# SobeyMIL/MVOC

Hardware: AMD Instinct MI355X
Metric: UNet3D denoising steps/sec, 16x512^2 frames, inversion+compose (higher is better)
Workload: dtype f16

## Files before the change

### mvoc_amd/csrc/attention.hip

```cpp
#include <stdlib.h>

#include "common.h"

namespace {

typedef __fp16 fp16x4_t __attribute__((__vector_size__(4 * sizeof(__fp16))));
template <int D> struct FlashPitch { static constexpr int K = 2 * D + 16, V = D == 64 ? 192 : 320; };

struct AttnArgs {
  const half_t *q, *k, *v;
  half_t* out;
  long q_bs, q_ts, k_bs, k_ts, v_bs, v_ts, o_bs, o_ts;
  int nbatch, heads, tq, tk, kv_bdiv, causal;
  float scale_log2;
  long v2_off, o2_off;
  int qblocks;
};

__device__ __forceinline__ int vt_slot_group(int key) {
  return ((((key >> 5) * 2 + ((key >> 4) & 1)) * 2) + ((key >> 2) & 1));
}
__device__ __forceinline__ int vt_slot_elem(int key) { return ((key >> 3) & 1) * 4 + (key & 3); }

constexpr float FLASH_THR = 8.0f;

typedef float f32x2 __attribute__((ext_vector_type(2)));
__device__ __forceinline__ float flash_xhalf_max(float x) {
  const unsigned u = __builtin_bit_cast(unsigned, x);
  const auto sw = __builtin_amdgcn_permlane32_swap(u, u, false, false);
  return fmaxf(__builtin_bit_cast(float, (unsigned)sw[0]), __builtin_bit_cast(float, (unsigned)sw[1]));
}

template <int D, int NV>
#ifndef FLASH_MINW
#define FLASH_MINW 4
#endif
__global__ __launch_bounds__(256, (D == 64 && NV == 1) ? FLASH_MINW : 1) void flash_kernel(const AttnArgs p) {
  constexpr int KPITCH = FlashPitch<D>::K, VPITCH = FlashPitch<D>::V;
  constexpr int ND = D / 16, NT = D / 32, CPK = D / 8, NCH = 64 * CPK / 256;
  __shared__ __attribute__((aligned(16))) char smem[64 * KPITCH + NV * 64 * VPITCH];
  char* Ks = smem;
  char* Vs = smem + 64 * KPITCH;
  const int tid = threadIdx.x, lane = tid & 63;
  const int wave = __builtin_amdgcn_readfirstlane(tid >> 6);
  const int r = lane & 31, h = lane >> 5;
  const unsigned logical = xcd_remap(blockIdx.x, gridDim.x);
  const unsigned qb_ = logical % (unsigned)p.qblocks, hb_ = logical / (unsigned)p.qblocks;
  const int head = (int)(hb_ % (unsigned)p.heads), b = (int)(hb_ / (unsigned)p.heads);
  const int q0 = (int)qb_ * 128 + wave * 32;

  const half_t* qp = p.q + (long)b * p.q_bs + head * D;
  const int qrow = min(q0 + r, p.tq - 1);
  half8_t qf[ND];
#pragma unroll
  for (int s = 0; s < ND; ++s) qf[s] = *reinterpret_cast<const half8_t*>(qp + (long)qrow * p.q_ts + 16 * s + 8 * h);

  const char* kb = reinterpret_cast<const char*>(p.k + (long)(b / p.kv_bdiv) * p.k_bs + head * D);
  const char* vb = reinterpret_cast<const char*>(p.v + (long)(b / p.kv_bdiv) * p.v_bs + head * D);
  const unsigned k_rb = (unsigned)p.k_ts * 2u, v_rb = (unsigned)p.v_ts * 2u;
  unsigned koff[NCH], voff[NCH];
#pragma unroll
  for (int i = 0; i < NCH; ++i) {
    const int c = tid + i * 256;
    koff[i] = (unsigned)(c / CPK) * k_rb + (unsigned)(c % CPK) * 16u;
    voff[i] = (unsigned)(c / CPK) * v_rb + (unsigned)(c % CPK) * 16u;
  }

  f32x16 ot[NV][NT];
#pragma unroll
  for (int v = 0; v < NV; ++v)
#pragma unroll
    for (int dt = 0; dt < NT; ++dt)
#pragma unroll
      for (int e = 0; e < 16; ++e) ot[v][dt][e] = 0.f;
  float mrun = -INFINITY, lrun = 0.f;

  const int ntiles = (p.tk + 63) / 64;
  half8_t kreg[NCH], vreg[NV][NCH];
  auto gload = [&](int kt) {
    const char* kt_ = kb + (size_t)kt * 64u * k_rb;
    const char* vt_ = vb + (size_t)kt * 64u * v_rb;
    const bool ragged = __builtin_amdgcn_readfirstlane(kt * 64 + 64 > p.tk);
#pragma unroll
    for (int i = 0; i < NCH; ++i) {
      unsigned ko = koff[i], vo = voff[i];
      if (ragged) {
        const int c = tid + i * 256;
        const unsigned row = (unsigned)min(c / CPK, p.tk - 1 - kt * 64);
        ko = row * k_rb + (unsigned)(c % CPK) * 16u;
        vo = row * v_rb + (unsigned)(c % CPK) * 16u;
      }
      kreg[i] = *reinterpret_cast<const half8_t*>(kt_ + ko);
#pragma unroll
      for (int v = 0; v < NV; ++v) vreg[v][i] = *reinterpret_cast<const half8_t*>(vt_ + (size_t)v * (size_t)p.v2_off * 2u + vo);
    }
  };
  gload(0);
  for (int kt = 0; kt < ntiles; ++kt) {
    __syncthreads();
#pragma unroll
    for (int i = 0; i < NCH; ++i) {
      const int c = tid + i * 256;
      const int key = c / CPK, dc = c % CPK;
      *reinterpret_cast<half8_t*>(Ks + key * KPITCH + dc * 16) = kreg[i];
#pragma unroll
      for (int v = 0; v < NV; ++v)
        *reinterpret_cast<half8_t*>(Vs + v * 64 * VPITCH + key * VPITCH + dc * 16) = vreg[v][i];
    }
    __syncthreads();
    if (kt + 1 < ntiles) gload(kt + 1);

    f32x16 st[2];
#pragma unroll
    for (int t = 0; t < 2; ++t) {
#pragma unroll
      for (int e = 0; e < 16; ++e) st[t][e] = 0.f;
#pragma unroll
      for (int s = 0; s < ND; ++s) {
        const half8_t kf = *reinterpret_cast<const half8_t*>(Ks + (32 * t + r) * KPITCH + (16 * s + 8 * h) * 2);
        st[t] = __builtin_amdgcn_mfma_f32_32x32x16_f16(kf, qf[s], st[t], 0, 0, 0);
      }
    }
    if (__builtin_amdgcn_readfirstlane((kt == ntiles - 1) && (p.tk & 63))) {
#pragma unroll
      for (int t = 0; t < 2; ++t)
#pragma unroll
        for (int e = 0; e < 16; ++e)
          if (kt * 64 + 32 * t + 8 * (e >> 2) + 4 * h + (e & 3) >= p.tk) st[t][e] = -INFINITY;
    }
    if (p.causal) {
#pragma unroll
      for (int t = 0; t < 2; ++t)
#pragma unroll
        for (int e = 0; e < 16; ++e)
          if (kt * 64 + 32 * t + 8 * (e >> 2) + 4 * h + (e & 3) > q0 + r) st[t][e] = -INFINITY;
    }
    float mx = st[0][0];
#pragma unroll
    for (int t = 0; t < 2; ++t)
#pragma unroll
      for (int e = 0; e < 16; ++e) mx = fmaxf(mx, st[t][e]);
    mx = flash_xhalf_max(mx);
    if (__any((mx - mrun) * p.scale_log2 > FLASH_THR)) {
      const float mnew = fmaxf(mrun, mx);
      const float alpha = __builtin_amdgcn_exp2f((mrun - mnew) * p.scale_log2);
      mrun = mnew;
      lrun *= alpha;
#pragma unroll
      for (int v = 0; v < NV; ++v)
#pragma unroll
        for (int dt = 0; dt < NT; ++dt)
#pragma unroll
          for (int e = 0; e < 16; ++e) ot[v][dt][e] *= alpha;
    }
    const f32x2 sc2 = {p.scale_log2, p.scale_log2}, mc2 = {-mrun * p.scale_log2, -mrun * p.scale_log2};
#pragma unroll
    for (int t = 0; t < 2; ++t)
#pragma unroll
      for (int e = 0; e < 16; e += 2) {
        const f32x2 a = __builtin_elementwise_fma(f32x2{st[t][e], st[t][e + 1]}, sc2, mc2);
        st[t][e] = __builtin_amdgcn_exp2f(a[0]);
        st[t][e + 1] = __builtin_amdgcn_exp2f(a[1]);
      }

#pragma unroll
    for (int t = 0; t < 2; ++t)
#pragma unroll
      for (int s = 0; s < 2; ++s) {
        half8_t pf;
#pragma unroll
        for (int j = 0; j < 8; ++j) pf[j] = (half_t)st[t][8 * s + j];
#pragma unroll
        for (int j = 0; j < 4; ++j) lrun = __builtin_amdgcn_fdot2(half2_t{pf[2 * j], pf[2 * j + 1]}, half2_t{(half_t)1.f, (half_t)1.f}, lrun, false);
        const int krow = 32 * t + 16 * s + 4 * h + ((lane & 15) >> 2);
#pragma unroll
        for (int v = 0; v < NV; ++v)
#pragma unroll
          for (int dt = 0; dt < NT; ++dt) {
            const char* va = Vs + v * 64 * VPITCH + krow * VPITCH + (32 * dt + 16 * ((lane >> 4) & 1) + 4 * (lane & 3)) * 2;
            const fp16x4_t lo = __builtin_amdgcn_ds_read_tr16_b64_v4f16((__attribute__((address_space(3))) fp16x4_t*)va);
            const fp16x4_t hi = __builtin_amdgcn_ds_read_tr16_b64_v4f16((__attribute__((address_space(3))) fp16x4_t*)(va + 8 * VPITCH));
            half8_t vf;
#pragma unroll
            for (int e = 0; e < 4; ++e) {
              vf[e] = (half_t)lo[e];
              vf[4 + e] = (half_t)hi[e];
            }
            ot[v][dt] = __builtin_amdgcn_mfma_f32_32x32x16_f16(vf, pf, ot[v][dt], 0, 0, 0);
          }
      }
  }
  const float ltot = lrun + __shfl_xor(lrun, 32);
  const float inv = 1.0f / ltot;
  int lane_e = tid;
  asm volatile("" : "+v"(lane_e));
  const int r_e = lane_e & 31, h_e = (lane_e >> 5) & 1;
  if (q0 + r_e < p.tq) {
#pragma unroll
    for (int v = 0; v < NV; ++v) {
      half_t* op = p.out + v * p.o2_off + (long)b * p.o_bs + (long)(q0 + r_e) * p.o_ts + head * D;
#pragma unroll
      for (int dt = 0; dt < NT; ++dt)
#pragma unroll
        for (int q = 0; q < 4; ++q) {
          half4_t o;
#pragma unroll
          for (int e = 0; e < 4; ++e) o[e] = (half_t)(ot[v][dt][q * 4 + e] * inv);
          *reinterpret_cast<half4_t*>(op + 32 * dt + 8 * q + 4 * h_e) = o;
        }
    }
  }
}

#define F3_BAR()                         \
  do {                                   \
    __builtin_amdgcn_sched_barrier(0);   \
    __builtin_amdgcn_s_barrier();        \
    __builtin_amdgcn_sched_barrier(0);   \
  } while (0)
#define F3_FENCE() __builtin_amdgcn_sched_barrier(0)
#define F3_GRP(V, T)                                   \
  do {                                                 \
    __builtin_amdgcn_sched_group_barrier(0x008, 1, 0); \
    __builtin_amdgcn_sched_group_barrier(0x002, V, 0); \
    __builtin_amdgcn_sched_group_barrier(0x400, T, 0); \
  } while (0)
#define F3_RD(R) __builtin_amdgcn_sched_group_barrier(0x100, R, 0)
#ifdef MVOC_F3_STAMPS
__device__ unsigned long long f3_dbg[8];
#define F3_STAMP(i)                                                                      \
  do {                                                                                   \
    unsigned long long t_;                                                               \
    asm volatile("s_memtime %0\n\ts_waitcnt lgkmcnt(0)" : "=s"(t_)::"memory");          \
    if (blockIdx.x == 0 && tid == 0) { f3_acc[i] += t_ - f3_last; }                      \
    f3_last = t_;                                                                        \
  } while (0)
#else
#define F3_STAMP(i)
#endif
typedef unsigned u32x4 __attribute__((ext_vector_type(4)));
__device__ __forceinline__ void f3_dma(const u32x4 rsrc, unsigned voff, unsigned lds) {
  unsigned keep;
  asm volatile("s_mov_b32 %0, m0\n\ts_mov_b32 m0, %2\n\ts_nop 0\n\tbuffer_load_dwordx4 %1, %3, 0 offen lds\n\ts_mov_b32 m0, %0"
               : "=&s"(keep) : "v"(voff), "s"(lds), "s"(rsrc) : "memory");
}
__device__ __forceinline__ u32x4 f3_rsrc(const void* base, unsigned bytes) {
  const unsigned long long a = (unsigned long long)base;
  u32x4 r;
  r[0] = __builtin_amdgcn_readfirstlane((unsigned)a);
  r[1] = __builtin_amdgcn_readfirstlane((unsigned)(a >> 32));
  r[2] = __builtin_amdgcn_readfirstlane(bytes);
  r[3] = 0x00020000u;
  return r;
}
template <int N>
__device__ __forceinline__ void f3_wait_vm() {
  asm volatile("s_waitcnt vmcnt(%0)" ::"n"(N) : "memory");
}
#ifndef F3_W1
#define F3_W1 3
#endif
template <int NV>
__global__ __launch_bounds__(256, NV == 1 ? F3_W1 : 2) void flash3_kernel(const AttnArgs p) {
  constexpr int D = 64, NS = (NV == 1 && F3_W1 == 2) ? 4 : 3, TILE = 8192 * (1 + NV), PCS = 2 + 2 * NV;
  __shared__ __attribute__((aligned(1024))) char smem[NS * TILE];
#ifdef MVOC_F3_STAMPS
  unsigned long long f3_acc[6] = {0, 0, 0, 0, 0, 0}, f3_last = 0, f3_t0, f3_r0;
#endif
  const int tid = threadIdx.x, lane = tid & 63;
  const int wave = __builtin_amdgcn_readfirstlane(tid >> 6);
  const int r = lane & 31, h = lane >> 5;
#ifdef MVOC_F3_STAMPS
  asm volatile("s_memtime %0\n\ts_memrealtime %1\n\ts_waitcnt lgkmcnt(0)" : "=s"(f3_t0), "=s"(f3_r0)::"memory");
  f3_last = f3_t0;
#endif
  const unsigned logical = xcd_remap(blockIdx.x, gridDim.x);
  const unsigned qb_ = logical % (unsigned)p.qblocks, hb_ = logical / (unsigned)p.qblocks;
  const int head = (int)(hb_ % (unsigned)p.heads), b = (int)(hb_ / (unsigned)p.heads);
  const int q0 = (int)qb_ * 128 + wave * 32;
  const int nt = (p.tk + 63) >> 6;

  const unsigned k_rb = (unsigned)p.k_ts * 2u, v_rb = (unsigned)p.v_ts * 2u;
  const half_t* kb = p.k + (long)(b / p.kv_bdiv) * p.k_bs + head * D;
  const half_t* vb = p.v + (long)(b / p.kv_bdiv) * p.v_bs + head * D;
  const u32x4 rs_k = f3_rsrc(kb, (unsigned)(p.tk - 1) * k_rb + 128u);
  const u32x4 rs_v0 = f3_rsrc(vb, (unsigned)(p.tk - 1) * v_rb + 128u);
  const u32x4 rs_v1 = f3_rsrc(vb + p.v2_off, (unsigned)(p.tk - 1) * v_rb + 128u);
  unsigned ksrc[2], vsrc[2];
#pragma unroll
  for (int j = 0; j < 2; ++j) {
    const int key_l = 16 * wave + 8 * j + (lane >> 3), pc = lane & 7;
    ksrc[j] = (unsigned)key_l * k_rb + (unsigned)((pc ^ ((key_l >> 1) & 7)) * 16);
    vsrc[j] = (unsigned)key_l * v_rb + (unsigned)((pc ^ (((key_l >> 1) & 1) << 2)) * 16);
  }
  const unsigned ktile = 64u * k_rb, vtile = 64u * v_rb;
  const unsigned lds0 = (unsigned)(size_t)(__attribute__((address_space(3))) char*)smem;
  auto issue = [&](int tile, int so) {
    const unsigned base = lds0 + (unsigned)so + (unsigned)wave * 2048u;
#pragma unroll
    for (int j = 0; j < 2; ++j) f3_dma(rs_k, ksrc[j] + (unsigned)tile * ktile, base + j * 1024);
#pragma unroll
    for (int v = 0; v < NV; ++v)
#pragma unroll
      for (int j = 0; j < 2; ++j) f3_dma(v ? rs_v1 : rs_v0, vsrc[j] + (unsigned)tile * vtile, base + 8192 * (1 + v) + j * 1024);
  };
  const half_t* qp = p.q + (long)b * p.q_bs + head * D;
  const int qrow = min(q0 + r, p.tq - 1);
  half8_t qf[4];
#pragma unroll
  for (int s = 0; s < 4; ++s) qf[s] = *reinterpret_cast<const half8_t*>(qp + (long)qrow * p.q_ts + 16 * s + 8 * h);
  asm volatile("s_nop 4" ::: "memory");
  F3_FENCE();
#pragma unroll
  for (int t = 0; t < NS - 1; ++t) issue(t, t * TILE);
  F3_FENCE();

  f32x16 ot[NV][2];
#pragma unroll
  for (int v = 0; v < NV; ++v)
#pragma unroll
    for (int dt = 0; dt < 2; ++dt)
#pragma unroll
      for (int e = 0; e < 16; ++e) ot[v][dt][e] = 0.f;
  float mrun = -INFINITY, lrun = 0.f;
  f32x16 sa[2], sb[2];
  f32x16 zero16;
#pragma unroll
  for (int e = 0; e < 16; ++e) zero16[e] = 0.f;

  int kfo[4];
#pragma unroll
  for (int s = 0; s < 4; ++s) kfo[s] = r * 128 + (((2 * s + h) ^ ((r >> 1) & 7)) * 16);
  const int vq = (lane & 15) >> 2;
  int vfo[2];
#pragma unroll
  for (int dt = 0; dt < 2; ++dt) vfo[dt] = 8192 + (4 * h + vq) * 128 + (((32 * ((lane >> 4) & 1) + 8 * (lane & 3))) | ((dt ^ ((vq >> 1) & 1)) << 6));

  f3_wait_vm<(NS - 2) * PCS>();
  F3_BAR();
#pragma unroll
  for (int t = 0; t < 2; ++t) {
    sa[t] = zero16;
#pragma unroll
    for (int s = 0; s < 4; ++s) {
      const half8_t kf = *reinterpret_cast<const half8_t*>(smem + kfo[s] + 4096 * t);
      sa[t] = __builtin_amdgcn_mfma_f32_32x32x16_f16(kf, qf[s], sa[t], 0, 0, 0);
    }
  }
  int o_v = 0, o_k = TILE, o_w = (NS - 1) * TILE;

  auto body = [&](f32x16(&cur)[2], f32x16(&nxt)[2], const int t) {
    F3_STAMP(4);
    f3_wait_vm<(NS - 3) * PCS>();
    F3_BAR();
    F3_STAMP(0);
    issue(t + NS - 1, o_w);
    F3_FENCE();
    F3_STAMP(1);
    const char* Kn = smem + o_k;
    const char* Vc = smem + o_v;
    if (__builtin_amdgcn_readfirstlane((t == nt - 1) && (p.tk & 63))) {
#pragma unroll
      for (int tt = 0; tt < 2; ++tt)
#pragma unroll
        for (int e = 0; e < 16; ++e)
          if (t * 64 + 32 * tt + 8 * (e >> 2) + 4 * h + (e & 3) >= p.tk) cur[tt][e] = -INFINITY;
    }
    F3_FENCE();
    half8_t kf[2][4];
#pragma unroll
    for (int s = 0; s < 2; ++s)
#pragma unroll
      for (int tt = 0; tt < 2; ++tt) kf[tt][s] = *reinterpret_cast<const half8_t*>(Kn + kfo[s] + 4096 * tt);
    half8_t pf[2];
    half8_t vf[3][NV][2];
    auto vread = [&](const int f) {
#pragma unroll
      for (int v = 0; v < NV; ++v)
#pragma unroll
        for (int dt = 0; dt < 2; ++dt) {
          const char* va = Vc + 8192 * v + vfo[dt] + (32 * (f >> 1) + 16 * (f & 1)) * 128;
          const fp16x4_t lo = __builtin_amdgcn_ds_read_tr16_b64_v4f16((__attribute__((address_space(3))) fp16x4_t*)va);
          const fp16x4_t hi = __builtin_amdgcn_ds_read_tr16_b64_v4f16((__attribute__((address_space(3))) fp16x4_t*)(va + 8 * 128));
#pragma unroll
          for (int e = 0; e < 4; ++e) {
            vf[f % 3][v][dt][e] = (half_t)lo[e];
            vf[f % 3][v][dt][4 + e] = (half_t)hi[e];
          }
        }
    };
    vread(0);
    F3_FENCE();
    auto smma = [&](const int i) {
      const int tt = i & 1, s_ = i >> 1;
      nxt[tt] = __builtin_amdgcn_mfma_f32_32x32x16_f16(kf[tt][s_], qf[s_], s_ == 0 ? zero16 : nxt[tt], 0, 0, 0);
    };
    auto pvmma = [&](const int f, const int dt) {
#pragma unroll
      for (int v = 0; v < NV; ++v) ot[v][dt] = __builtin_amdgcn_mfma_f32_32x32x16_f16(vf[f % 3][v][dt], pf[f & 1], ot[v][dt], 0, 0, 0);
    };
    float mx = fmaxf(cur[0][0], cur[0][1]);
#pragma unroll
    for (int tt = 0; tt < 2; ++tt)
#pragma unroll
      for (int e = tt ? 0 : 2; e < 16; e += 2) mx = __builtin_fmaxf(__builtin_fmaxf(mx, cur[tt][e]), cur[tt][e + 1]);
    smma(0); smma(1); smma(2);
    if constexpr (NV == 2) smma(3);
    mx = flash_xhalf_max(mx);
    if constexpr (NV == 1) { F3_GRP(6, 0); F3_GRP(6, 0); F3_GRP(6, 0); }
    else { F3_GRP(4, 0); F3_GRP(5, 0); F3_GRP(4, 0); F3_GRP(5, 0); }
    F3_STAMP(2);
    if (__any((mx - mrun) * p.scale_log2 > FLASH_THR)) {
      const float mnew = fmaxf(mrun, mx);
      const float alpha = __builtin_amdgcn_exp2f((mrun - mnew) * p.scale_log2);
      mrun = mnew;
      lrun *= alpha;
#pragma unroll
      for (int v = 0; v < NV; ++v)
#pragma unroll
        for (int dt = 0; dt < 2; ++dt)
#pragma unroll
          for (int e = 0; e < 16; ++e) ot[v][dt][e] *= alpha;
    }
    F3_FENCE();
    const f32x2 sc2 = {p.scale_log2, p.scale_log2}, mc2 = {-mrun * p.scale_log2, -mrun * p.scale_log2};
#pragma unroll
    for (int s = 2; s < 4; ++s)
#pragma unroll
      for (int tt = 0; tt < 2; ++tt) kf[tt][s] = *reinterpret_cast<const half8_t*>(Kn + kfo[s] + 4096 * tt);
#pragma unroll
    for (int f = 0; f < 4; ++f) {
      const int tt = f >> 1, s_ = f & 1;
      if (f < 3) vread(f + 1);
      half8_t& pn = pf[f & 1];
      float x[8];
#pragma unroll
      for (int j = 0; j < 8; j += 2) {
        const f32x2 a = __builtin_elementwise_fma(f32x2{cur[tt][8 * s_ + j], cur[tt][8 * s_ + j + 1]}, sc2, mc2);
        x[j] = __builtin_amdgcn_exp2f(a[0]);
        x[j + 1] = __builtin_amdgcn_exp2f(a[1]);
      }
#pragma unroll
      for (int j = 0; j < 8; ++j) pn[j] = (half_t)x[j];
#pragma unroll
      for (int j = 0; j < 4; ++j) lrun = __builtin_amdgcn_fdot2(half2_t{pn[2 * j], pn[2 * j + 1]}, half2_t{(half_t)1.f, (half_t)1.f}, lrun, false);
      if (f == 0) {
        smma(NV == 1 ? 3 : 4); smma(NV == 1 ? 4 : 5);
        if constexpr (NV == 2) { smma(6); smma(7); } else smma(5);
      } else {
        pvmma(f - 1, 0); pvmma(f - 1, 1);
        if constexpr (NV == 1) { if (f < 3) smma(5 + f); }
      }
    }
    pvmma(3, 0);
    pvmma(3, 1);
    if constexpr (NV == 1) {
      F3_RD(8); F3_GRP(5, 3); F3_GRP(5, 2); F3_GRP(5, 3);
      F3_RD(4); F3_GRP(5, 2); F3_GRP(5, 3); F3_GRP(5, 2);
      F3_RD(4); F3_GRP(5, 3); F3_GRP(5, 2); F3_GRP(5, 3);
      F3_GRP(5, 2); F3_GRP(5, 3); F3_GRP(5, 2); F3_GRP(5, 2);
    } else {
      F3_RD(12); F3_GRP(3, 2); F3_GRP(3, 2); F3_GRP(3, 2); F3_GRP(3, 2);
      F3_RD(8); F3_GRP(3, 2); F3_GRP(3, 2); F3_GRP(3, 2); F3_GRP(3, 2);
      F3_RD(8); F3_GRP(3, 2); F3_GRP(3, 2); F3_GRP(3, 2); F3_GRP(3, 2);
      F3_GRP(3, 2); F3_GRP(3, 2); F3_GRP(3, 2); F3_GRP(3, 2);
      F3_GRP(3, 0); F3_GRP(3, 0); F3_GRP(3, 0); F3_GRP(3, 0);
    }
    F3_FENCE();
    F3_STAMP(3);
    const int o_ = o_v; o_v = o_k;
    o_k = o_k + TILE == NS * TILE ? 0 : o_k + TILE;
    o_w = o_;
  };
#pragma unroll 1
  for (int t = 0;; t += 2) {
    body(sa, sb, t);
    if (t + 1 >= nt) break;
    body(sb, sa, t + 1);
    if (t + 2 >= nt) break;
  }
  f3_wait_vm<0>();
#ifdef MVOC_F3_STAMPS
  if (blockIdx.x == 0 && tid == 0) {
    unsigned long long t1_, r1_;
    asm volatile("s_memtime %0\n\ts_memrealtime %1\n\ts_waitcnt lgkmcnt(0)" : "=s"(t1_), "=s"(r1_)::"memory");
    for (int i = 0; i < 5; ++i) f3_dbg[i] = f3_acc[i];
    f3_dbg[5] = t1_ - f3_t0;
    f3_dbg[7] = r1_ - f3_r0;
    f3_dbg[6] = (unsigned long long)nt;
  }
#endif

  const float ltot = lrun + __shfl_xor(lrun, 32);
  const float inv = 1.0f / ltot;
  if (q0 + r < p.tq) {
#pragma unroll
    for (int v = 0; v < NV; ++v) {
      half_t* op = p.out + v * p.o2_off + (long)b * p.o_bs + (long)(q0 + r) * p.o_ts + head * D;
#pragma unroll
      for (int dt = 0; dt < 2; ++dt)
#pragma unroll
        for (int q = 0; q < 4; ++q) {
          half4_t o;
#pragma unroll
          for (int e = 0; e < 4; ++e) o[e] = (half_t)(ot[v][dt][q * 4 + e] * inv);
          *reinterpret_cast<half4_t*>(op + 32 * dt + 8 * q + 4 * h) = o;
        }
    }
  }
}
#undef F3_BAR
#undef F3_FENCE
#undef F3_GRP
#undef F3_RD
#undef F3_STAMP

struct TAttnArgs {
  const half_t *q, *k, *v;
  half_t* out;
  long q_bs, q_ps, q_ts, k_bs, k_ps, k_ts, v_bs, v_ps, v_ts, o_bs, o_ps, o_ts;
  int nsample, hw, heads, frames;
  int logf, logp, pgroups;
  long ntask;
  float scale_log2;
};

constexpr int TVPITCH = 64;

__global__ __launch_bounds__(256) void tattn_kernel(const TAttnArgs p) {
  __shared__ __attribute__((aligned(16))) char smem[4 * 64 * TVPITCH];
  const int tid = threadIdx.x, lane = tid & 63, wave = tid >> 6;
  const int r = lane & 31, h = lane >> 5;
  char* Vs = smem + wave * 64 * TVPITCH;
  const int F = p.frames, logf = p.logf, P = 1 << p.logp;
  const long task = (long)blockIdx.x * 4 + wave;
  const bool active = task < p.ntask;
  const long tk = active ? task : p.ntask - 1;
  const int head = (int)(tk % p.heads);
  const long bp = tk / p.heads;
  const long smp = bp / p.pgroups, px0 = (bp % p.pgroups) << p.logp;
  const half8_t zero8 = {0, 0, 0, 0, 0, 0, 0, 0};
  auto row_px = [&](int row) { return (long)(P > 1 ? row >> logf : 0); };
  auto row_fr = [&](int row) { return P > 1 ? row & (F - 1) : row; };
  auto row_ok = [&](int row) { return (P > 1 || row < F) && px0 + row_px(row) < p.hw; };

  const half_t* qb = p.q + smp * p.q_bs + px0 * p.q_ps + head * 64;
  const half_t* kb = p.k + smp * p.k_bs + px0 * p.k_ps + head * 64;
  const half_t* vb = p.v + smp * p.v_bs + px0 * p.v_ps + head * 64;

#pragma unroll
  for (int i = 0; i < 4; ++i) {
    const int c = lane + 64 * i;
    const int key = c >> 3, dc = c & 7;
    half8_t vr = zero8;
    if (row_ok(key)) vr = *reinterpret_cast<const half8_t*>(vb + row_px(key) * p.v_ps + (long)row_fr(key) * p.v_ts + dc * 8);
    const int g = (((key >> 4) & 1) * 2) + ((key >> 2) & 1), j = vt_slot_elem(key);
#pragma unroll
    for (int e = 0; e < 8; ++e) {
      const int d = dc * 8 + e;
      *reinterpret_cast<half_t*>(Vs + d * TVPITCH + ((g ^ ((d >> 3) & 3)) * 16) + j * 2) = vr[e];
    }
  }
  f32x16 st;
#pragma unroll
  for (int e = 0; e < 16; ++e) st[e] = 0.f;
  const bool rok = row_ok(r);
  const long koff = row_px(r) * p.k_ps + (long)row_fr(r) * p.k_ts, qoff = row_px(r) * p.q_ps + (long)row_fr(r) * p.q_ts;
#pragma unroll
  for (int s = 0; s < 4; ++s) {
    half8_t kf = zero8, qf = zero8;
    if (rok) {
      kf = *reinterpret_cast<const half8_t*>(kb + koff + 16 * s + 8 * h);
      qf = *reinterpret_cast<const half8_t*>(qb + qoff + 16 * s + 8 * h);
    }
    st = __builtin_amdgcn_mfma_f32_32x32x16_f16(kf, qf, st, 0, 0, 0);
  }
  float mx = -INFINITY;
#pragma unroll
  for (int e = 0; e < 16; ++e) {
    const int key = 8 * (e >> 2) + 4 * h + (e & 3);
    const bool ok = P > 1 ? (key >> logf) == (r >> logf) : key < F;
    const float sv = ok ? st[e] * p.scale_log2 : -INFINITY;
    st[e] = sv;
    mx = fmaxf(mx, sv);
  }
  mx = fmaxf(mx, __shfl_xor(mx, 32));
  float ps = 0.f;
#pragma unroll
  for (int e = 0; e < 16; ++e) {
    const float pv = __builtin_amdgcn_exp2f(st[e] - mx);
    st[e] = pv;
    ps += pv;
  }
  ps += __shfl_xor(ps, 32);
  const float inv = 1.0f / ps;

  __syncthreads();
  f32x16 ot[2];
#pragma unroll
  for (int dt = 0; dt < 2; ++dt)
#pragma unroll
    for (int e = 0; e < 16; ++e) ot[dt][e] = 0.f;
#pragma unroll
  for (int s = 0; s < 2; ++s) {
    half8_t pf;
#pragma unroll
    for (int j = 0; j < 8; ++j) pf[j] = (half_t)st[8 * s + j];
    const int g = s * 2 + h;
#pragma unroll
    for (int dt = 0; dt < 2; ++dt) {
      const int d = 32 * dt + r;
      const half8_t vf = *reinterpret_cast<const half8_t*>(Vs + d * TVPITCH + ((g ^ ((d >> 3) & 3)) * 16));
      ot[dt] = __builtin_amdgcn_mfma_f32_32x32x16_f16(vf, pf, ot[dt], 0, 0, 0);
    }
  }
  if (active && rok) {
    half_t* op = p.out + smp * p.o_bs + (px0 + row_px(r)) * p.o_ps + (long)row_fr(r) * p.o_ts + head * 64;
#pragma unroll
    for (int dt = 0; dt < 2; ++dt)
#pragma unroll
      for (int q = 0; q < 4; ++q) {
        half4_t o;
#pragma unroll
        for (int e = 0; e < 4; ++e) o[e] = (half_t)(ot[dt][q * 4 + e] * inv);
        *reinterpret_cast<half4_t*>(op + 32 * dt + 8 * q + 4 * h) = o;
      }
  }
}

}

static const int g_f3_env = getenv("MVOC_FLASH3") ? atoi(getenv("MVOC_FLASH3")) : -1;

extern "C" int mvoc_flash_attn_f16(const mvoc_attn_desc* d, void* stream) {
  MVOC_REQUIRE(d && d->q && d->k && d->v && d->out, -1, "flash_attn: null operand");
  MVOC_REQUIRE(d->nbatch > 0 && d->heads > 0 && d->tq > 0 && d->tk > 0, -1, "flash_attn: empty problem");
  MVOC_REQUIRE(d->nbatch <= 65535 && d->heads <= 65535, -2, "flash_attn: grid too large");
  MVOC_REQUIRE(d->q_ts % 8 == 0 && d->k_ts % 8 == 0 && d->v_ts % 8 == 0 && d->o_ts % 4 == 0, -2,
               "flash_attn: row strides must keep 16-byte alignment");
  AttnArgs a;
  a.q = (const half_t*)d->q; a.k = (const half_t*)d->k; a.v = (const half_t*)d->v; a.out = (half_t*)d->out;
  a.q_bs = d->q_bs; a.q_ts = d->q_ts; a.k_bs = d->k_bs; a.k_ts = d->k_ts; a.v_bs = d->v_bs; a.v_ts = d->v_ts;
  a.o_bs = d->o_bs; a.o_ts = d->o_ts;
  a.nbatch = d->nbatch; a.heads = d->heads; a.tq = d->tq; a.tk = d->tk; a.kv_bdiv = d->kv_bdiv > 0 ? d->kv_bdiv : 1;
  const int hd = d->head_dim > 0 ? d->head_dim : 64;
  MVOC_REQUIRE(hd == 64 || hd == 96, -2, "flash_attn: head_dim (%d) must be 64 or 96", hd);
  MVOC_REQUIRE(!d->causal || d->tq == d->tk, -2, "flash_attn: the causal form is self-attention (tq == tk)");
  a.causal = d->causal;
  a.scale_log2 = (d->scale > 0.f ? d->scale : (hd == 64 ? 0.125f : 1.0f / sqrtf((float)hd))) * 1.4426950408889634f;
  hipStream_t s = (hipStream_t)stream;
  MvocProfScope prof(MVOC_FAM_FLASH, s, (d->v2 ? 2.0 : 1.0) * 4.0 * d->nbatch * d->heads * (double)d->tq * d->tk * hd);
  a.qblocks = (d->tq + 127) / 128;
  const long nblk = (long)a.qblocks * d->heads * d->nbatch;
  MVOC_REQUIRE(nblk < 0x7fffffffL, -2, "flash_attn: grid too large");
  dim3 grid((unsigned)nblk);
  a.v2_off = a.o2_off = 0;
  MVOC_REQUIRE(d->pipelined >= 0 && d->pipelined <= 2, -1, "flash_attn: pipelined must be 0 (by key count), 1 (never) or 2 (wherever it applies)");
  const int f3_mode = d->pipelined ? d->pipelined - 1 : g_f3_env;
  const bool pipelined = hd == 64 && !d->causal && (f3_mode >= 0 ? f3_mode != 0 : d->tk >= 2048);
  if (d->v2) {
    MVOC_REQUIRE(d->out2 && hd == 64, -2, "flash_attn: the paired form needs out2 and head_dim 64");
    a.v2_off = (const half_t*)d->v2 - a.v;
    a.o2_off = (half_t*)d->out2 - a.out;
    MVOC_REQUIRE(a.v2_off % 8 == 0 && a.o2_off % 4 == 0, -2, "flash_attn: v2 / out2 must keep 16-byte alignment");
    if (pipelined) hipLaunchKernelGGL((flash3_kernel<2>), grid, dim3(256), 0, s, a);
    else hipLaunchKernelGGL((flash_kernel<64, 2>), grid, dim3(256), 0, s, a);
  } else if (hd == 64) {
    if (pipelined) hipLaunchKernelGGL((flash3_kernel<1>), grid, dim3(256), 0, s, a);
    else hipLaunchKernelGGL((flash_kernel<64, 1>), grid, dim3(256), 0, s, a);
  } else {
    hipLaunchKernelGGL((flash_kernel<96, 1>), grid, dim3(256), 0, s, a);
  }
  return mvoc_check_launch("flash_kernel");
}

#ifdef MVOC_F3_STAMPS
extern "C" int mvoc_f3_stamps_read(unsigned long long* host8) {
  return hipMemcpyFromSymbol(host8, HIP_SYMBOL(f3_dbg), sizeof(unsigned long long) * 8) == hipSuccess ? 0 : -1;
}
#endif

extern "C" int mvoc_temporal_attn_f16(const mvoc_tattn_desc* d, void* stream) {
  MVOC_REQUIRE(d && d->q && d->k && d->v && d->out, -1, "temporal_attn: null operand");
  MVOC_REQUIRE(d->nsample > 0 && d->hw > 0 && d->heads > 0, -1, "temporal_attn: empty problem");
  MVOC_REQUIRE(d->frames >= 1 && d->frames <= 32, -2, "temporal_attn: frames (%d) must be in [1, 32]", d->frames);
  MVOC_REQUIRE(d->q_ts % 8 == 0 && d->k_ts % 8 == 0 && d->v_ts % 8 == 0 && d->o_ts % 4 == 0 && d->q_ps % 8 == 0 &&
                   d->k_ps % 8 == 0 && d->v_ps % 8 == 0 && d->o_ps % 4 == 0,
               -2, "temporal_attn: strides must keep 16-byte alignment");
  TAttnArgs a;
  a.q = (const half_t*)d->q; a.k = (const half_t*)d->k; a.v = (const half_t*)d->v; a.out = (half_t*)d->out;
  a.q_bs = d->q_bs; a.q_ps = d->q_ps; a.q_ts = d->q_ts; a.k_bs = d->k_bs; a.k_ps = d->k_ps; a.k_ts = d->k_ts;
  a.v_bs = d->v_bs; a.v_ps = d->v_ps; a.v_ts = d->v_ts; a.o_bs = d->o_bs; a.o_ps = d->o_ps; a.o_ts = d->o_ts;
  a.nsample = d->nsample; a.hw = d->hw; a.heads = d->heads; a.frames = d->frames;
  a.logf = d->frames == 8 ? 3 : d->frames == 16 ? 4 : 5;
  a.logp = d->frames == 8 ? 2 : d->frames == 16 ? 1 : 0;
  a.pgroups = (d->hw + (1 << a.logp) - 1) >> a.logp;
  a.ntask = (long)d->nsample * a.pgroups * d->heads;
  a.scale_log2 = 0.125f * 1.4426950408889634f;
  const long nblk = (a.ntask + 3) / 4;
  MVOC_REQUIRE(nblk < 0x7fffffffL, -2, "temporal_attn: grid too large");
  hipStream_t s = (hipStream_t)stream;
  MvocProfScope prof(MVOC_FAM_TATTN, s, 4.0 * (double)d->nsample * d->hw * d->heads * d->frames * 64 * 2);
  hipLaunchKernelGGL(tattn_kernel, dim3((unsigned)nblk), dim3(256), 0, s, a);
  return mvoc_check_launch("tattn_kernel");
}
```

Measured before the change: 24.96.

## Add persistent software-pipelined temporal attention kernel with LDS-staged coalesced I/O

Adds tattn2_kernel, a persistent kernel whose grid is capped at CU count times three blocks. Each wave loops over tasks and double-buffers register fragments, loading the next task's Q/K/V while computing the current one. Q/K reads and output writes go through a per-wave LDS staging area so global accesses are row-coalesced, and non-temporal loads are used when the working set is large. It is enabled by default for 8 or 16 frames. The cost is extra LDS traffic and wave-level fences, and the register pressure of two fragment buffers may reduce occupancy.

```diff
diff --git a/mvoc_amd/csrc/attention.hip b/mvoc_amd/csrc/attention.hip
--- a/mvoc_amd/csrc/attention.hip
+++ b/mvoc_amd/csrc/attention.hip
@@ -625,6 +625,176 @@
         for (int e = 0; e < 4; ++e) o[e] = (half_t)(ot[dt][q * 4 + e] * inv);
         *reinterpret_cast<half4_t*>(op + 32 * dt + 8 * q + 4 * h) = o;
       }
+  }
+}
+
+constexpr int TATTN2_BLOCKS_PER_CU = 3;
+constexpr int TRPITCH = 144;
+constexpr int TATTN2_WAVE_LDS = 64 * TVPITCH + 32 * TRPITCH;
+struct TAttn2Frag { half8_t k[4], q[4], v[4]; };
+
+__device__ __forceinline__ float tattn2_xhalf_max(float x) {
+  const unsigned u = __builtin_bit_cast(unsigned, x);
+  const auto sw = __builtin_amdgcn_permlane32_swap(u, u, false, false);
+  return fmaxf(__builtin_bit_cast(float, (unsigned)sw[0]), __builtin_bit_cast(float, (unsigned)sw[1]));
+}
+__device__ __forceinline__ float tattn2_xhalf_sum(float x) {
+  const unsigned u = __builtin_bit_cast(unsigned, x);
+  const auto sw = __builtin_amdgcn_permlane32_swap(u, u, false, false);
+  return __builtin_bit_cast(float, (unsigned)sw[0]) + __builtin_bit_cast(float, (unsigned)sw[1]);
+}
+__device__ __forceinline__ void tattn2_lds_fence() {
+  __builtin_amdgcn_fence(__ATOMIC_RELEASE, "wavefront");
+  __builtin_amdgcn_wave_barrier();
+  __builtin_amdgcn_fence(__ATOMIC_ACQUIRE, "wavefront");
+}
+
+template <bool NT>
+__global__ __launch_bounds__(256, TATTN2_BLOCKS_PER_CU) void tattn2_kernel(const TAttnArgs p) {
+  __shared__ __attribute__((aligned(16))) char smem[4 * TATTN2_WAVE_LDS];
+  const int tid = threadIdx.x, lane = tid & 63, wave = __builtin_amdgcn_readfirstlane(tid >> 6);
+  const int r = lane & 31, h = lane >> 5;
+  char* Vs = smem + wave * TATTN2_WAVE_LDS;
+  char* Rs = Vs + 64 * TVPITCH;
+  const int F = p.frames, logf = p.logf;
+  const unsigned nw = gridDim.x * 4u, ntask = (unsigned)p.ntask;
+  const int rpx = r >> logf, dc = lane & 7, rb = lane >> 3;
+  const long klane = (long)rb * p.k_ts + dc * 8, qlane = (long)rb * p.q_ts + dc * 8, olane = (long)rb * p.o_ts + dc * 8;
+  char* rrow = Rs + rb * TRPITCH + dc * 16;
+  const char* rfrag = Rs + r * TRPITCH + 16 * h;
+  char* rout = Rs + r * TRPITCH + 8 * h;
+  const int vg = (lane >> 3) & 3, jh = lane >> 5;
+  const int vkey = 16 * (vg >> 1) + 8 * jh + 4 * (vg & 1), vpx = vkey >> logf;
+  const long voff = vpx * p.v_ps + (long)(vkey & (F - 1)) * p.v_ts + dc * 8, voff0 = voff - vpx * p.v_ps;
+  char* vdst = Vs + dc * 8 * TVPITCH + ((vg ^ (dc & 3)) * 16) + jh * 8;
+  const half8_t zero8 = {0, 0, 0, 0, 0, 0, 0, 0};
+  const half4_t zero4 = {0, 0, 0, 0};
+
+  auto ld16 = [](const half_t* src) {
+    const half8_t* s8 = reinterpret_cast<const half8_t*>(src);
+    return NT ? __builtin_nontemporal_load(s8) : *s8;
+  };
+  auto load = [&](unsigned tk, TAttn2Frag& f) {
+    const unsigned head = tk % (unsigned)p.heads, bp = tk / (unsigned)p.heads;
+    const long smp = bp / (unsigned)p.pgroups, px0 = (long)(bp % (unsigned)p.pgroups) << p.logp;
+    const half_t* qb = p.q + smp * p.q_bs + px0 * p.q_ps + head * 64;
+    const half_t* kb = p.k + smp * p.k_bs + px0 * p.k_ps + head * 64;
+    const half_t* vb = p.v + smp * p.v_bs + px0 * p.v_ps + head * 64 + (px0 + vpx < p.hw ? voff : voff0);
+#pragma unroll
+    for (int i = 0; i < 4; ++i) {
+      const int px = (8 * i) >> logf, fr = (8 * i) & (F - 1);
+      const long pxl = px0 + px < p.hw ? px : 0;
+      f.k[i] = ld16(kb + pxl * p.k_ps + (long)fr * p.k_ts + klane);
+      f.q[i] = ld16(qb + pxl * p.q_ps + (long)fr * p.q_ts + qlane);
+    }
+#pragma unroll
+    for (int i = 0; i < 4; ++i) f.v[i] = ld16(vb + (long)i * p.v_ts);
+  };
+
+  auto compute = [&](unsigned tk, const TAttn2Frag& f) {
+    const unsigned head = tk % (unsigned)p.heads, bp = tk / (unsigned)p.heads;
+    const long smp = bp / (unsigned)p.pgroups, px0 = (long)(bp % (unsigned)p.pgroups) << p.logp;
+    const bool vok = px0 + vpx < p.hw;
+#pragma unroll
+    for (int e = 0; e < 8; ++e) {
+      const half4_t w = {f.v[0][e], f.v[1][e], f.v[2][e], f.v[3][e]};
+      *reinterpret_cast<half4_t*>(vdst + e * TVPITCH) = vok ? w : zero4;
+    }
+    half8_t kf[4], qf[4];
+#pragma unroll
+    for (int i = 0; i < 4; ++i)
+      *reinterpret_cast<half8_t*>(rrow + 8 * i * TRPITCH) = px0 + ((8 * i) >> logf) < p.hw ? f.k[i] : zero8;
+    tattn2_lds_fence();
+#pragma unroll
+    for (int s = 0; s < 4; ++s) kf[s] = *reinterpret_cast<const half8_t*>(rfrag + 32 * s);
+    tattn2_lds_fence();
+#pragma unroll
+    for (int i = 0; i < 4; ++i)
+      *reinterpret_cast<half8_t*>(rrow + 8 * i * TRPITCH) = px0 + ((8 * i) >> logf) < p.hw ? f.q[i] : zero8;
+    tattn2_lds_fence();
+#pragma unroll
+    for (int s = 0; s < 4; ++s) qf[s] = *reinterpret_cast<const half8_t*>(rfrag + 32 * s);
+    tattn2_lds_fence();
+    f32x16 st;
+#pragma unroll
+    for (int e = 0; e < 16; ++e) st[e] = 0.f;
+#pragma unroll
+    for (int s = 0; s < 4; ++s) st = __builtin_amdgcn_mfma_f32_32x32x16_f16(kf[s], qf[s], st, 0, 0, 0);
+    float mx = -INFINITY;
+#pragma unroll
+    for (int e = 0; e < 16; ++e) {
+      const int key = 8 * (e >> 2) + 4 * h + (e & 3);
+      const bool ok = (key >> logf) == rpx;
+      const float sv = ok ? st[e] * p.scale_log2 : -INFINITY;
+      st[e] = sv;
+      mx = fmaxf(mx, sv);
+    }
+    mx = tattn2_xhalf_max(mx);
+    float ps = 0.f;
+#pragma unroll
+    for (int e = 0; e < 16; ++e) {
+      const float pv = __builtin_amdgcn_exp2f(st[e] - mx);
+      st[e] = pv;
+      ps += pv;
+    }
+    ps = tattn2_xhalf_sum(ps);
+    const float inv = 1.0f / ps;
+
+    f32x16 ot[2];
+#pragma unroll
+    for (int dt = 0; dt < 2; ++dt)
+#pragma unroll
+      for (int e = 0; e < 16; ++e) ot[dt][e] = 0.f;
+#pragma unroll
+    for (int s = 0; s < 2; ++s) {
+      half8_t pf;
+#pragma unroll
+      for (int j = 0; j < 8; ++j) pf[j] = (half_t)st[8 * s + j];
+      const int g = s * 2 + h;
+#pragma unroll
+      for (int dt = 0; dt < 2; ++dt) {
+        const int d = 32 * dt + r;
+        const half8_t vf = *reinterpret_cast<const half8_t*>(Vs + d * TVPITCH + ((g ^ ((d >> 3) & 3)) * 16));
+        ot[dt] = __builtin_amdgcn_mfma_f32_32x32x16_f16(vf, pf, ot[dt], 0, 0, 0);
+      }
+    }
+#pragma unroll
+    for (int dt = 0; dt < 2; ++dt)
+#pragma unroll
+      for (int q = 0; q < 4; ++q) {
+        half4_t o;
+#pragma unroll
+        for (int e = 0; e < 4; ++e) o[e] = (half_t)(ot[dt][q * 4 + e] * inv);
+        *reinterpret_cast<half4_t*>(rout + 64 * dt + 16 * q) = o;
+      }
+    tattn2_lds_fence();
+    half_t* ob = p.out + smp * p.o_bs + px0 * p.o_ps + head * 64 + olane;
+#pragma unroll
+    for (int i = 0; i < 4; ++i) {
+      const int px = (8 * i) >> logf, fr = (8 * i) & (F - 1);
+      const half8_t o = *reinterpret_cast<const half8_t*>(rrow + 8 * i * TRPITCH);
+      if (px0 + px < p.hw) *reinterpret_cast<half8_t*>(ob + px * p.o_ps + (long)fr * p.o_ts) = o;
+    }
+    tattn2_lds_fence();
+  };
+
+  unsigned task = blockIdx.x * 4u + wave;
+  if (task >= ntask) return;
+  TAttn2Frag fa, fb;
+  load(task, fa);
+  for (;;) {
+    unsigned nxt = task + nw;
+    load(nxt < ntask ? nxt : task, fb);
+    __builtin_amdgcn_sched_barrier(0);
+    compute(task, fa);
+    if (nxt >= ntask) break;
+    task = nxt;
+    nxt = task + nw;
+    load(nxt < ntask ? nxt : task, fa);
+    __builtin_amdgcn_sched_barrier(0);
+    compute(task, fb);
+    if (nxt >= ntask) break;
+    task = nxt;
   }
 }
 
@@ -680,6 +850,20 @@
 }
 #endif
 
+static const int g_tattn2_env = getenv("MVOC_TATTN2") ? atoi(getenv("MVOC_TATTN2")) : 1;
+
+static int tattn2_cus() {
+  static int cached[64] = {0};
+  int dev = 0;
+  if (hipGetDevice(&dev) != hipSuccess || dev < 0 || dev >= 64) return 0;
+  if (cached[dev] == 0) {
+    int n = 0;
+    if (hipDeviceGetAttribute(&n, hipDeviceAttributeMultiprocessorCount, dev) != hipSuccess) return 0;
+    cached[dev] = n;
+  }
+  return cached[dev];
+}
+
 extern "C" int mvoc_temporal_attn_f16(const mvoc_tattn_desc* d, void* stream) {
   MVOC_REQUIRE(d && d->q && d->k && d->v && d->out, -1, "temporal_attn: null operand");
   MVOC_REQUIRE(d->nsample > 0 && d->hw > 0 && d->heads > 0, -1, "temporal_attn: empty problem");
@@ -701,6 +885,16 @@
   MVOC_REQUIRE(nblk < 0x7fffffffL, -2, "temporal_attn: grid too large");
   hipStream_t s = (hipStream_t)stream;
   MvocProfScope prof(MVOC_FAM_TATTN, s, 4.0 * (double)d->nsample * d->hw * d->heads * d->frames * 64 * 2);
+  if (g_tattn2_env != 0 && (d->frames == 8 || d->frames == 16) && a.ntask < 0x7fffffffL) {
+    const int cus = tattn2_cus();
+    MVOC_REQUIRE(cus > 0, -3, "temporal_attn: cannot read the device's compute unit count");
+    const long cap = (long)cus * TATTN2_BLOCKS_PER_CU;
+    const dim3 grid((unsigned)(nblk < cap ? nblk : cap));
+    static const long nt_min = getenv("MVOC_TATTN2_NT_BYTES") ? atol(getenv("MVOC_TATTN2_NT_BYTES")) : (256L << 20);
+    if (3L * d->nsample * d->hw * d->heads * d->frames * 64 * 2 >= nt_min) hipLaunchKernelGGL(tattn2_kernel<true>, grid, dim3(256), 0, s, a);
+    else hipLaunchKernelGGL(tattn2_kernel<false>, grid, dim3(256), 0, s, a);
+    return mvoc_check_launch("tattn2_kernel");
+  }
   hipLaunchKernelGGL(tattn_kernel, dim3((unsigned)nblk), dim3(256), 0, s, a);
   return mvoc_check_launch("tattn_kernel");
 }
```

Result: no change. 25.16, median of 6 (+0.8%).
